# mauro3/KissMCMC.jl

Hardware: AMD Instinct MI355X
Metric: walker-steps/sec (higher is better)
Workload: dtype f64

## Files before the change

### include/kissmcmc_hip.h

```cpp
#ifndef KISSMCMC_HIP_H
#define KISSMCMC_HIP_H

#include <stdint.h>

#ifdef __cplusplus
extern "C" {
#endif

#define KMC_VERSION 100

typedef enum kmc_status {
    KMC_OK = 0,
    KMC_ERR_A_SCALE = 1,
    KMC_ERR_ODD_WALKERS = 2,
    KMC_ERR_TOO_FEW_WALKERS = 3,
    KMC_ERR_BAD_ARG = 4,
    KMC_ERR_NONFINITE_LOGP = 5,
    KMC_ERR_HIP = 6,
    KMC_ERR_OOM = 7,
    KMC_ERR_NO_DEVICE = 8,
    KMC_ERR_UNSUPPORTED = 9
} kmc_status;

typedef enum kmc_density {
// ... 344 lines not shown
                                 int device, double* mean, double* cov, int64_t* n_out, int64_t* info);
kmc_status  kmc_cov_plan(int64_t ncols, int32_t* tile_cols, int32_t* strip_tiles, int32_t* nstrips, int32_t* rows_per_wave_block);
kmc_status  kmc_cov_correlation(int64_t ncols, const double* cov, double* corr, double* sd);

kmc_status  kmc_sampler_pointwise_stats(kmc_sampler* s, int64_t first_sample, const uint8_t* walker_mask ,
                                        int64_t thin, const double* data , int64_t ndata2, int32_t ncols2,
                                        double* stats, int64_t* n_out, int64_t* info);
kmc_status  kmc_chain_pointwise_stats(kmc_user_density* density, const double* params, const double* chain_host ,
                                      int64_t nsamples, int64_t nwalkers, int64_t ndim, int64_t first_sample, const uint8_t* walker_mask,
                                      int64_t thin, const double* data, int64_t ndata2, int32_t ncols2, int device, double* stats,
                                      int64_t* n_out, int64_t* info);
kmc_status  kmc_sampler_pointwise_loglike(kmc_sampler* s, int64_t first_sample, const uint8_t* walker_mask, int64_t thin, const double* data,
                                          int64_t ndata2, int32_t ncols2, int64_t obs_first, int64_t obs_count, double* out, int64_t* n_out);
kmc_status  kmc_chain_pointwise_loglike(kmc_user_density* density, const double* params, const double* chain_host, int64_t nsamples,
                                        int64_t nwalkers, int64_t ndim, int64_t first_sample, const uint8_t* walker_mask, int64_t thin,
                                        const double* data, int64_t ndata2, int32_t ncols2, int64_t obs_first, int64_t obs_count, int device,
                                        double* out, int64_t* n_out);
kmc_status  kmc_pointwise_plan(int64_t n, int64_t ndata, int64_t* run_len, int64_t* nruns, int32_t* lanes_per_run, int32_t* slots,
                               int64_t* nwaves);
kmc_status  kmc_waic_stats(int64_t J, int64_t n, const double* stats, double* lppd_j, double* p_waic_j, double* elpd_j, double* totals);

kmc_status  kmc_sampler_psis_loo(kmc_sampler* s, int64_t first_sample, const uint8_t* walker_mask , int64_t thin,
                                 double r_eff, int64_t obs_first, int64_t obs_count, int64_t workspace_bytes, double* stats, double* lppd_j,
                                 int64_t* n_out, int64_t* info);
kmc_status  kmc_chain_psis_loo(kmc_user_density* density, const double* params, const double* chain_host ,
                               int64_t nsamples, int64_t nwalkers, int64_t ndim, int64_t first_sample, const uint8_t* walker_mask, int64_t thin,
                               double r_eff, int64_t obs_first, int64_t obs_count, int64_t workspace_bytes, int device, double* stats,
                               double* lppd_j, int64_t* n_out, int64_t* info);
kmc_status  kmc_sampler_psis_tail(kmc_sampler* s, int64_t first_sample, const uint8_t* walker_mask, int64_t thin, double r_eff, int64_t obs_first,
                                  int64_t obs_count, int64_t workspace_bytes, double* tail, double* m_j, double* xc_j, int32_t* n_tail_j,
                                  int64_t* tail_len, int64_t* n_out);
kmc_status  kmc_chain_psis_tail(kmc_user_density* density, const double* params, const double* chain_host, int64_t nsamples, int64_t nwalkers,
                                int64_t ndim, int64_t first_sample, const uint8_t* walker_mask, int64_t thin, double r_eff, int64_t obs_first,
                                int64_t obs_count, int64_t workspace_bytes, int device, double* tail, double* m_j, double* xc_j,
                                int32_t* n_tail_j, int64_t* tail_len, int64_t* n_out);
kmc_status  kmc_psis_plan(int64_t n, int64_t ndata, double r_eff, int64_t workspace_bytes, int64_t* tail_len, int64_t* m_est,
                          int64_t* obs_per_block, int64_t* passes);
kmc_status  kmc_loo_stats(int64_t J, int64_t n, const double* stats, const double* lppd_j, double* p_loo_j, double* totals);
kmc_status  kmc_psis_smooth_host(int64_t nt, const double* x, double xc, double* k_hat, double* sigma, double* s, double* sums);

kmc_status  kmc_sampler_relative_eff(kmc_sampler* s, int64_t first_sample, const uint8_t* walker_mask , int64_t thin,
                                     int64_t obs_first, int64_t obs_count, int32_t split, int64_t max_lag, int64_t workspace_bytes,
                                     double* r_eff_j, double* ess_j, int64_t* T_j, int32_t* flags_j, int64_t* m_out, int64_t* h_out, int64_t* n_out,
                                     int64_t* info);
kmc_status  kmc_chain_relative_eff(kmc_user_density* density, const double* params, const double* chain_host ,
                                   int64_t nsamples, int64_t nwalkers, int64_t ndim, int64_t first_sample, const uint8_t* walker_mask, int64_t thin,
                                   int64_t obs_first, int64_t obs_count, int32_t split, int64_t max_lag, int64_t workspace_bytes, int device,
                                   double* r_eff_j, double* ess_j, int64_t* T_j, int32_t* flags_j, int64_t* m_out, int64_t* h_out, int64_t* n_out,
                                   int64_t* info);
kmc_status  kmc_sampler_pointwise_weights(kmc_sampler* s, int64_t first_sample, const uint8_t* walker_mask, int64_t thin, const double* data,
                                          int64_t ndata2, int32_t ncols2, int64_t obs_first, int64_t obs_count, double* v, double* M_j,
                                          int64_t* n_out);
kmc_status  kmc_chain_pointwise_weights(kmc_user_density* density, const double* params, const double* chain_host, int64_t nsamples,
                                        int64_t nwalkers, int64_t ndim, int64_t first_sample, const uint8_t* walker_mask, int64_t thin,
                                        const double* data, int64_t ndata2, int32_t ncols2, int64_t obs_first, int64_t obs_count, int device,
                                        double* v, double* M_j, int64_t* n_out);
kmc_status  kmc_sampler_psis_loo_reff(kmc_sampler* s, int64_t first_sample, const uint8_t* walker_mask, int64_t thin,
                                      const double* r_eff_j , int32_t split, int64_t max_lag, int64_t obs_first,
                                      int64_t obs_count, int64_t workspace_bytes, double* stats, double* lppd_j, double* r_eff_used,
                                      int64_t* tail_len_j, int64_t* n_reff_nan, int64_t* n_out, int64_t* info);
kmc_status  kmc_chain_psis_loo_reff(kmc_user_density* density, const double* params, const double* chain_host, int64_t nsamples, int64_t nwalkers,
                                    int64_t ndim, int64_t first_sample, const uint8_t* walker_mask, int64_t thin, const double* r_eff_j,
                                    int32_t split, int64_t max_lag, int64_t obs_first, int64_t obs_count, int64_t workspace_bytes, int device,
                                    double* stats, double* lppd_j, double* r_eff_used, int64_t* tail_len_j, int64_t* n_reff_nan, int64_t* n_out,
                                    int64_t* info);
kmc_status  kmc_sampler_psis_tail_reff(kmc_sampler* s, int64_t first_sample, const uint8_t* walker_mask, int64_t thin, const double* r_eff_j,
                                       int32_t split, int64_t max_lag, int64_t obs_first, int64_t obs_count, int64_t workspace_bytes, double* tail,
                                       double* m_j, double* xc_j, int32_t* n_tail_j, int64_t* tail_len, double* r_eff_used, int64_t* tail_len_j,
                                       int64_t* n_reff_nan, int64_t* n_out);
kmc_status  kmc_chain_psis_tail_reff(kmc_user_density* density, const double* params, const double* chain_host, int64_t nsamples, int64_t nwalkers,
                                     int64_t ndim, int64_t first_sample, const uint8_t* walker_mask, int64_t thin, const double* r_eff_j,
                                     int32_t split, int64_t max_lag, int64_t obs_first, int64_t obs_count, int64_t workspace_bytes, int device,
                                     double* tail, double* m_j, double* xc_j, int32_t* n_tail_j, int64_t* tail_len, double* r_eff_used,
                                     int64_t* tail_len_j, int64_t* n_reff_nan, int64_t* n_out);

kmc_status  kmc_debug_accept_terms(uint64_t seed, uint64_t step, uint64_t walker0, int64_t n, int64_t nhalf, double a_scale,
                                   int64_t ndim, int device, int64_t* partner_host, double* z_host, double* t1_host, double* lu_host);
kmc_status  kmc_debug_chain_by_walker(const void* src_host, int is_float, int64_t K, int64_t nl, int64_t ld, int64_t nd, int64_t w0,
                                      int64_t nw, int64_t dst_stride, double* dst_host, int64_t dst_len, int device);
kmc_status  kmc_debug_rows_compact(const double* src_host, int64_t rows, int64_t ld, int64_t nd, double* dst_host, int64_t dst_len,
                                   int device);
int         kmc_debug_phase_spec(int density, int L, int K, int iter);
int         kmc_debug_shared_draws(int density, int L, int K, int iter);
int         kmc_debug_replay_variant(int density, int64_t nwalkers, int64_t ndim, int64_t nburnin, int64_t g0, int64_t n, int moments, int chain);

#ifdef __cplusplus
}
#endif
#endif
```

### kissmcmc.jl_amd/_lib.py

```python
from __future__ import annotations

import ctypes as C
import os

_HERE = os.path.dirname(os.path.abspath(__file__))
LIB_PATH = os.environ.get("KMC_LIB_PATH") or os.path.join(_HERE, "libkissmcmc_hip.so")

OK, ERR_A_SCALE, ERR_ODD_WALKERS, ERR_TOO_FEW_WALKERS, ERR_BAD_ARG, ERR_NONFINITE_LOGP, \
    ERR_HIP, ERR_OOM, ERR_NO_DEVICE, ERR_UNSUPPORTED = range(10)
GAUSSIAN_ISO, EXPONENTIAL, ROSENBROCK, LOGNORMAL, MVNORMAL2 = range(5)
USER_DENSITY = 100
HOST_DENSITY = 101
DATA_DENSITY = 102
HOST_LOGPDF_FN = C.CFUNCTYPE(C.c_int, C.POINTER(C.c_double), C.c_int64, C.c_int64, C.POINTER(C.c_double), C.c_void_p)
HOST_PROPOSE_FN = C.CFUNCTYPE(C.c_int, C.POINTER(C.c_double), C.c_int64, C.c_int64, C.POINTER(C.c_double), C.c_void_p)
HOST_ACCEPTED_FN = C.CFUNCTYPE(C.c_int, C.POINTER(C.c_uint8), C.c_int64, C.c_int64, C.c_int64, C.c_int32, C.c_void_p)
F64 = 0
F32 = 1
STORE_CHAIN, STORE_LOGP, MOMENTS, NO_GRAPH, P2P, ISLANDS, P2P_FINEGRAINED, P2P_PUSH = 1, 2, 4, 8, 16, 64, 128, 512
STREAM_CHAIN = 2048
CHAIN_BY_WALKER = 4096
STORE_BLOBS = 8192
MOVE_STRETCH, MOVE_DE, MOVE_SNOOKER, MOVE_MIX = 0, 1, 3, 4
MIX_MAX = 4
TEMPS_MAX = 64
CONV_NEED_LAGS, CONV_TRUNCATED = 1, 2
CONV_HAS_NAN = 4
TEMPER_WHOLE, TEMPER_LIKELIHOOD = 0, 1
P2P_HANDLE_BYTES = 128
RCCL_ID_BYTES = 128

SYMBOLS = [
    "kmc_version", "kmc_device_count", "kmc_last_error", "kmc_status_string", "kmc_validate",
    "kmc_g_pdf", "kmc_cdf_g_inv", "kmc_emcee_run", "kmc_sampler_create", "kmc_sampler_destroy",
    "kmc_sampler_set_stream", "kmc_sampler_bind_positions", "kmc_sampler_p2p_export", "kmc_sampler_p2p_connect", "kmc_sampler_p2p_connect_local", "kmc_sampler_p2p_link_probe", "kmc_sampler_set_positions", "kmc_sampler_init_ball", "kmc_sampler_set_state", "kmc_sampler_run", "kmc_sampler_half_step",
    "kmc_sampler_sync", "kmc_sampler_last_run_ms", "kmc_sampler_generation", "kmc_sampler_nsamples",
    "kmc_sampler_launch_count", "kmc_sampler_describe", "kmc_sampler_device_ptr", "kmc_sampler_get_positions",
    "kmc_sampler_get_logp", "kmc_sampler_get_naccept", "kmc_sampler_get_accept_ratio",
    "kmc_sampler_get_moments", "kmc_sampler_get_chain", "kmc_sampler_get_chain_by_walker", "kmc_logpdf_eval", "kmc_logpdf_eval_host",
    "kmc_user_density_create", "kmc_user_density_create_body", "kmc_user_density_destroy", "kmc_metropolis_validate", "kmc_metropolis_run", "kmc_cholesky_lower", "kmc_int_acorr", "kmc_sampler_int_acorr",
    "kmc_sizeof_config", "kmc_sizeof_metropolis_config", "kmc_sizeof_outputs", "kmc_sizeof_metropolis_outputs", "kmc_deal_seed", "kmc_deal_perm", "kmc_sampler_deal_pack", "kmc_sampler_deal_unpack",
    "kmc_sampler_get_walker_ids", "kmc_sampler_set_walker_ids", "kmc_sampler_set_chain_host", "kmc_rccl_unique_id", "kmc_sampler_rccl_init",
    "kmc_sampler_rccl_capture", "kmc_sampler_rccl_set_capture", "kmc_rccl_version", "kmc_device_free_bytes",
    "kmc_sampler_launch_mode", "kmc_updated_budget", "kmc_set_updated_budget_mb", "kmc_debug_accept_terms",
    "kmc_debug_chain_by_walker", "kmc_debug_rows_compact", "kmc_debug_phase_spec", "kmc_debug_shared_draws", "kmc_debug_replay_variant",
    "kmc_user_density_create_body_blob", "kmc_user_density_nblob", "kmc_logpdf_blob_eval_host", "kmc_sampler_get_blobs",
    "kmc_device_cache_release", "kmc_user_density_is_separable", "kmc_host_prefault", "kmc_data_density_create",
    "kmc_sampler_get_rung_state", "kmc_sampler_set_rung_state", "kmc_sampler_get_swaps",
    "kmc_sampler_get_rung_loglike", "kmc_sampler_set_rung_loglike_sum", "kmc_sampler_get_ladder", "kmc_sampler_set_ladder",
    "kmc_sampler_order_stats", "kmc_sampler_chain_argmax", "kmc_chain_order_stats", "kmc_chain_argmax",
    "kmc_sampler_histograms", "kmc_chain_histograms", "kmc_hist_pair_plan",
    "kmc_sampler_lag_sums", "kmc_chain_lag_sums", "kmc_convergence_stats", "kmc_sampler_convergence", "kmc_chain_convergence",
    "kmc_convergence_plan",
    "kmc_rank_plan", "kmc_rank_normal_scores", "kmc_sampler_rank_scores", "kmc_chain_rank_scores", "kmc_sampler_rank_convergence",
    "kmc_chain_rank_convergence",
    "kmc_sampler_hdi", "kmc_chain_hdi", "kmc_hdi_span",
    "kmc_sampler_covariance", "kmc_chain_covariance", "kmc_cov_plan", "kmc_cov_correlation",
    "kmc_sampler_pointwise_stats", "kmc_chain_pointwise_stats", "kmc_sampler_pointwise_loglike", "kmc_chain_pointwise_loglike",
    "kmc_pointwise_plan", "kmc_waic_stats",
    "kmc_sampler_psis_loo", "kmc_chain_psis_loo", "kmc_sampler_psis_tail", "kmc_chain_psis_tail", "kmc_psis_plan", "kmc_loo_stats",
    "kmc_psis_smooth_host",
    "kmc_sampler_relative_eff", "kmc_chain_relative_eff", "kmc_sampler_pointwise_weights", "kmc_chain_pointwise_weights",
    "kmc_sampler_psis_loo_reff", "kmc_chain_psis_loo_reff", "kmc_sampler_psis_tail_reff", "kmc_chain_psis_tail_reff",
]


class Config(C.Structure):
    _fields_ = [
        ("dtype", C.c_int32),
        ("density", C.c_int32),
        ("params", C.c_double * 8),
        ("nwalkers", C.c_int64),
        ("ndim", C.c_int64),
        ("ngenerations", C.c_int64),
        ("nburnin", C.c_int64),
        ("nthin", C.c_int64),
        ("a_scale", C.c_double),
        ("seed", C.c_uint64),
        ("flags", C.c_uint32),
        ("device", C.c_int32),
        ("shard_rank", C.c_int32),
        ("shard_count", C.c_int32),
        ("user_density", C.c_void_p),
        ("island_gens", C.c_int32),
        ("island_size", C.c_int32),
        ("host_logpdf", C.c_void_p),
        ("host_user", C.c_void_p),
        ("host_accepted", C.c_void_p),
        ("deal_rank", C.c_int32),
        ("deal_count", C.c_int32),
        ("temper_mode", C.c_int32),
        ("temper_pad_", C.c_int32),
        ("adapt_until", C.c_int64),
        ("adapt_lag", C.c_double),
        ("adapt_time", C.c_double),
        ("adapt", C.c_int32),
        ("adapt_pad_", C.c_int32),
        ("snooker_gamma", C.c_double),
        ("mix_count", C.c_int32),
        ("mix_move0", C.c_int32), ("mix_move1", C.c_int32), ("mix_move2", C.c_int32), ("mix_move3", C.c_int32),
        ("mix_pad0_", C.c_int32), ("mix_pad1_", C.c_int32), ("mix_pad2_", C.c_int32),
        ("mix_weight0", C.c_double), ("mix_weight1", C.c_double), ("mix_weight2", C.c_double), ("mix_weight3", C.c_double),
        ("mix_gamma0", C.c_double), ("mix_gamma1", C.c_double), ("mix_gamma2", C.c_double), ("mix_gamma3", C.c_double),
        ("mix_sigma0", C.c_double), ("mix_sigma1", C.c_double), ("mix_sigma2", C.c_double), ("mix_sigma3", C.c_double),
        ("betas", C.c_void_p),
        ("ntemps", C.c_int32),
        ("swap_every", C.c_int32),
        ("move", C.c_int32),
        ("move_pad_", C.c_int32),
        ("de_gamma0", C.c_double),
        ("de_sigma", C.c_double),
    ]


class Outputs(C.Structure):
    _fields_ = [
        ("chain", C.POINTER(C.c_double)),
        ("chain_logp", C.POINTER(C.c_double)),
        ("accept_ratio", C.POINTER(C.c_double)),
        ("naccept", C.POINTER(C.c_int64)),
        ("final_pos", C.POINTER(C.c_double)),
        ("final_logp", C.POINTER(C.c_double)),
        ("sum", C.POINTER(C.c_double)),
        ("sumsq", C.POINTER(C.c_double)),
        ("nmoment", C.c_int64),
        ("nsamples", C.c_int64),
        ("device_ms", C.c_double),
        ("blobs", C.POINTER(C.c_double)),
# ... 147 lines not shown
    L.kmc_sampler_chain_argmax.argtypes = [vp, C.c_int64, bp, ip, ip, dp, dp]
    L.kmc_chain_order_stats.argtypes = [dp, dp, C.c_int64, C.c_int64, C.c_int64, C.c_int64, bp, ip, C.c_int32, C.c_int, dp, dp, ip]
    L.kmc_chain_argmax.argtypes = [dp, dp, C.c_int64, C.c_int64, C.c_int64, C.c_int64, bp, C.c_int, ip, ip, dp, dp]
    i32p = C.POINTER(C.c_int32)
    L.kmc_sampler_histograms.argtypes = [vp, C.c_int64, bp, i32p, C.c_int32, dp, C.c_int32, C.c_int32, ip, ip, ip, ip]
    L.kmc_chain_histograms.argtypes = [dp, dp, C.c_int64, C.c_int64, C.c_int64, C.c_int64, bp, i32p, C.c_int32, dp, C.c_int32, C.c_int, ip, ip, ip, ip]
    L.kmc_hist_pair_plan.argtypes = [C.c_int32, C.c_int32, i32p, i32p, i32p]
    L.kmc_sampler_lag_sums.argtypes = [vp, C.c_int64, bp, C.c_int32, C.c_int32, C.c_int64, C.c_int64, dp, dp, dp, ip, ip]
    L.kmc_chain_lag_sums.argtypes = [dp, dp, C.c_int64, C.c_int64, C.c_int64, C.c_int64, bp, C.c_int32, C.c_int64, C.c_int64, C.c_int, dp, dp, dp, ip, ip]
    L.kmc_convergence_stats.argtypes = [C.c_int64, C.c_int64, C.c_int64, dp, dp, dp, C.c_int64, C.c_int64, dp, dp, dp, dp, dp, dp, dp, ip, i32p]
    L.kmc_sampler_convergence.argtypes = [vp, C.c_int64, bp, C.c_int32, C.c_int32, C.c_int64, dp, dp, dp, dp, dp, dp, dp, ip, i32p, ip, ip, ip]
    L.kmc_chain_convergence.argtypes = [dp, dp, C.c_int64, C.c_int64, C.c_int64, C.c_int64, bp, C.c_int32, C.c_int64, C.c_int, dp, dp, dp, dp, dp, dp, dp, ip, i32p, ip, ip, ip]
    L.kmc_convergence_plan.argtypes = [i32p, i32p, i32p, i32p]
    L.kmc_rank_plan.argtypes = [i32p, i32p, i32p, i32p]
    L.kmc_rank_normal_scores.argtypes = [ip, C.c_int64, C.c_int64, dp]
    L.kmc_sampler_rank_scores.argtypes = [vp, C.c_int64, bp, C.c_int32, C.c_int32, C.c_int32, ip, dp, dp, ip, ip, ip]
    L.kmc_chain_rank_scores.argtypes = [dp, dp, C.c_int64, C.c_int64, C.c_int64, C.c_int64, bp, C.c_int32, C.c_int32, C.c_int, ip, dp, dp, ip, ip, ip]
    L.kmc_sampler_rank_convergence.argtypes = [vp, C.c_int64, bp, C.c_int32, C.c_int32, C.c_int64] + [dp] * 10 + [ip, i32p, ip, ip, ip]
    L.kmc_chain_rank_convergence.argtypes = [dp, dp, C.c_int64, C.c_int64, C.c_int64, C.c_int64, bp, C.c_int32, C.c_int64, C.c_int] + [dp] * 10 + [ip, i32p, ip, ip, ip]
    L.kmc_sampler_hdi.argtypes = [vp, C.c_int64, bp, C.c_int32, dp, C.c_int32, dp, dp, ip, ip, ip, ip]
    L.kmc_chain_hdi.argtypes = [dp, dp, C.c_int64, C.c_int64, C.c_int64, C.c_int64, bp, dp, C.c_int32, C.c_int, dp, dp, ip, ip, ip, ip]
    L.kmc_hdi_span.argtypes = [C.c_int64, C.c_double, ip, ip]
    L.kmc_sampler_covariance.argtypes = [vp, C.c_int64, bp, C.c_int32, dp, dp, ip, ip]
    L.kmc_chain_covariance.argtypes = [dp, dp, C.c_int64, C.c_int64, C.c_int64, C.c_int64, bp, C.c_int, dp, dp, ip, ip]
    L.kmc_cov_plan.argtypes = [C.c_int64, i32p, i32p, i32p, i32p]
    L.kmc_cov_correlation.argtypes = [C.c_int64, dp, dp, dp]
    held_out = [dp, C.c_int64, C.c_int32]
    host_chain = [vp, dp, dp, C.c_int64, C.c_int64, C.c_int64, C.c_int64, bp, C.c_int64]
    L.kmc_sampler_pointwise_stats.argtypes = [vp, C.c_int64, bp, C.c_int64] + held_out + [dp, ip, ip]
    L.kmc_chain_pointwise_stats.argtypes = host_chain + held_out + [C.c_int, dp, ip, ip]
    L.kmc_sampler_pointwise_loglike.argtypes = [vp, C.c_int64, bp, C.c_int64] + held_out + [C.c_int64, C.c_int64, dp, ip]
    L.kmc_chain_pointwise_loglike.argtypes = host_chain + held_out + [C.c_int64, C.c_int64, C.c_int, dp, ip]
    L.kmc_pointwise_plan.argtypes = [C.c_int64, C.c_int64, ip, ip, i32p, i32p, ip]
    L.kmc_waic_stats.argtypes = [C.c_int64, C.c_int64, dp, dp, dp, dp, dp]
    psis_sel = [C.c_double, C.c_int64, C.c_int64, C.c_int64]
    L.kmc_sampler_psis_loo.argtypes = [vp, C.c_int64, bp, C.c_int64] + psis_sel + [dp, dp, ip, ip]
    L.kmc_chain_psis_loo.argtypes = host_chain + psis_sel + [C.c_int, dp, dp, ip, ip]
    L.kmc_sampler_psis_tail.argtypes = [vp, C.c_int64, bp, C.c_int64] + psis_sel + [dp, dp, dp, i32p, ip, ip]
    L.kmc_chain_psis_tail.argtypes = host_chain + psis_sel + [C.c_int, dp, dp, dp, i32p, ip, ip]
    L.kmc_psis_plan.argtypes = [C.c_int64, C.c_int64, C.c_double, C.c_int64, ip, ip, ip, ip]
    L.kmc_loo_stats.argtypes = [C.c_int64, C.c_int64, dp, dp, dp, dp]
    L.kmc_psis_smooth_host.argtypes = [C.c_int64, dp, C.c_double, dp, dp, dp, dp]
    reff_sel = [C.c_int64, C.c_int64, C.c_int32, C.c_int64, C.c_int64]
    L.kmc_sampler_relative_eff.argtypes = [vp, C.c_int64, bp, C.c_int64] + reff_sel + [dp, dp, ip, i32p, ip, ip, ip, ip]
    L.kmc_chain_relative_eff.argtypes = host_chain + reff_sel + [C.c_int, dp, dp, ip, i32p, ip, ip, ip, ip]
    L.kmc_sampler_pointwise_weights.argtypes = [vp, C.c_int64, bp, C.c_int64] + held_out + [C.c_int64, C.c_int64, dp, dp, ip]
    L.kmc_chain_pointwise_weights.argtypes = host_chain + held_out + [C.c_int64, C.c_int64, C.c_int, dp, dp, ip]
    psis_reff = [dp, C.c_int32, C.c_int64, C.c_int64, C.c_int64, C.c_int64]
    L.kmc_sampler_psis_loo_reff.argtypes = [vp, C.c_int64, bp, C.c_int64] + psis_reff + [dp, dp, dp, ip, ip, ip, ip]
    L.kmc_chain_psis_loo_reff.argtypes = host_chain + psis_reff + [C.c_int, dp, dp, dp, ip, ip, ip, ip]
    L.kmc_sampler_psis_tail_reff.argtypes = [vp, C.c_int64, bp, C.c_int64] + psis_reff + [dp, dp, dp, i32p, ip, dp, ip, ip, ip]
    L.kmc_chain_psis_tail_reff.argtypes = host_chain + psis_reff + [C.c_int, dp, dp, dp, i32p, ip, dp, ip, ip, ip]
    L.kmc_deal_seed.restype = C.c_uint64
    L.kmc_deal_seed.argtypes = [C.c_uint64, C.c_int32]
    L.kmc_deal_perm.argtypes = [C.c_uint64, C.c_int64, C.c_int32, C.c_int64, ip, ip]
    L.kmc_sampler_deal_pack.argtypes = [vp, C.c_int64, vp]
    L.kmc_sampler_deal_unpack.argtypes = [vp, vp]
    L.kmc_sampler_get_walker_ids.argtypes = [vp, ip]
    L.kmc_sampler_set_walker_ids.argtypes = [vp, ip]
    L.kmc_sampler_set_chain_host.argtypes = [vp, dp, dp]
    L.kmc_rccl_unique_id.argtypes = [vp]
    L.kmc_sampler_rccl_init.argtypes = [vp, vp]
    L.kmc_sampler_rccl_capture.argtypes = [vp, C.POINTER(C.c_int)]
    L.kmc_sampler_rccl_set_capture.argtypes = [vp, C.c_int]
    L.kmc_rccl_version.argtypes = [C.POINTER(C.c_int), C.c_char_p, C.c_int64]
    L.kmc_device_free_bytes.argtypes = [C.c_int, C.POINTER(C.c_uint64), C.POINTER(C.c_uint64)]
    L.kmc_device_cache_release.argtypes = []
    L.kmc_device_cache_release.restype = None
    L.kmc_host_prefault.argtypes = [C.c_void_p, C.c_uint64, C.c_int]
    L.kmc_host_prefault.restype = None
    L.kmc_sampler_launch_mode.restype = C.c_int
    L.kmc_sampler_launch_mode.argtypes = [vp, C.POINTER(C.c_int)]
    L.kmc_updated_budget.restype = None
    L.kmc_updated_budget.argtypes = [ip, ip]
    L.kmc_set_updated_budget_mb.restype = None
    L.kmc_set_updated_budget_mb.argtypes = [C.c_double]
    L.kmc_debug_accept_terms.argtypes = [C.c_uint64, C.c_uint64, C.c_uint64, C.c_int64, C.c_int64, C.c_double, C.c_int64, C.c_int, ip, dp, dp, dp]
    L.kmc_debug_chain_by_walker.argtypes = [vp, C.c_int, C.c_int64, C.c_int64, C.c_int64, C.c_int64, C.c_int64, C.c_int64, C.c_int64, dp, C.c_int64, C.c_int]
    L.kmc_debug_rows_compact.argtypes = [dp, C.c_int64, C.c_int64, C.c_int64, dp, C.c_int64, C.c_int]
    L.kmc_debug_phase_spec.restype = C.c_int
    L.kmc_debug_phase_spec.argtypes = [C.c_int, C.c_int, C.c_int, C.c_int]
    L.kmc_debug_shared_draws.restype = C.c_int
    L.kmc_debug_shared_draws.argtypes = [C.c_int, C.c_int, C.c_int, C.c_int]
    L.kmc_debug_replay_variant.restype = C.c_int
    L.kmc_debug_replay_variant.argtypes = [C.c_int, C.c_int64, C.c_int64, C.c_int64, C.c_int64, C.c_int64, C.c_int, C.c_int]
    for fn, T in ((L.kmc_sizeof_config, Config), (L.kmc_sizeof_metropolis_config, MetropolisConfig),
                  (L.kmc_sizeof_outputs, Outputs), (L.kmc_sizeof_metropolis_outputs, MetropolisOutputs)):
        if fn() != C.sizeof(T):
            raise ImportError(f"{LIB_PATH}: struct layout mismatch ({fn.__name__}() = {fn()}, the ctypes mirror {T.__name__} is {C.sizeof(T)} bytes): "
                              "rebuild the library or update kissmcmc_jl_amd/_lib.py from include/kissmcmc_hip.h")
    _lib = L
    return L


def check(status: int) -> None:
    if status != OK:
        L = lib()
        msg = L.kmc_last_error().decode() or L.kmc_status_string(status).decode()
        raise KmcError(status, msg)
```

### kissmcmc.jl_amd/csrc/kmc_plan.hip

```cpp
#include <algorithm>
#include <cmath>
#include <cstdlib>
#include <cstring>

#include "kmc_sampler.hpp"

using namespace kmc;
using namespace kmc_host;

namespace kmc_host {
bool lookup(int density, int L, int K, int iter, bool p2p, bool ragged, bool f32, HalfStepFn* vec, HalfStepFn* gen)
{
    return with_density(density, false, [&](auto d) {
        using D = decltype(d);
        if (p2p && f32) { *vec = nullptr; *gen = nullptr; }
        else if (p2p) density_part<D, 2>(L, K, iter, ragged, false, vec, gen);
        else if (ragged || f32) density_part<D, 1>(L, K, iter, ragged, f32, vec, gen);
        else density_part<D, 0>(L, K, iter, false, false, vec, gen);
        return true;
    });
}

bool lookup_move(int move, int density, int L, int K, int iter, bool ragged, HalfStepFn* vec, HalfStepFn* gen)
{
    return with_density(density, false, [&](auto d) {
        if (move == KMC_MOVE_SNOOKER) density_part<decltype(d), 4>(L, K, iter, ragged, false, vec, gen);
        else if (move == KMC_MOVE_MIX) density_part<decltype(d), 5>(L, K, iter, ragged, false, vec, gen);
        else density_part<decltype(d), 3>(L, K, iter, ragged, false, vec, gen);
        return true;
    });
}

bool lookup_temper(int move, int density, int L, int K, int iter, bool ragged, HalfStepFn* vec, HalfStepFn* gen)
{
    return with_density(density, false, [&](auto d) {
        using D = decltype(d);
        if (move == KMC_MOVE_SNOOKER) temper_part<D, Move::Snooker>(L, K, iter, ragged, vec, gen);
        else if (move == KMC_MOVE_MIX) temper_part<D, Move::Mix>(L, K, iter, ragged, vec, gen);
        else if (move == KMC_MOVE_DE) temper_part<D, Move::DE>(L, K, iter, ragged, vec, gen);
        else temper_part<D, Move::Stretch>(L, K, iter, ragged, vec, gen);
        return true;
    });
}

HalfStepFn lookup_spec(int density, int L, int K, int iter)
{
    return with_density(density, HalfStepFn(nullptr), [&](auto d) { return spec_part<decltype(d)>(L, K, iter); });
}

HalfStepFn lookup_share(int density, int L, int K, int iter, int* share)
{
    *share = 0;
    return with_density(density, HalfStepFn(nullptr), [&](auto d) -> HalfStepFn {
        if constexpr (std::is_same<decltype(d), MvNormal2>::value) return nullptr;
        else return share_part<decltype(d)>(L, K, iter, share);
    });
}

LogpdfFn logpdf_fn(int density)
{
    return with_density(density, LogpdfFn(nullptr), [](auto d) { return logpdf_lookup<decltype(d)>(); });
}

bool resident_lane_wanted(int64_t ndim)
{
    std::string e;
    if (debug_opt("resident", &e) && e == "pair") return false;
    return ndim <= 8;
}
int lane_nd(int64_t ndim) { return (int)ndim; }

void philox_host(const uint32_t ctr[4], const uint32_t key[2], uint32_t out[4])
{
    uint32_t c0 = ctr[0], c1 = ctr[1], c2 = ctr[2], c3 = ctr[3], k0 = key[0], k1 = key[1];
    for (int r = 0; r < 10; ++r) {
        const uint64_t p0 = (uint64_t)0xD2511F53u * c0, p1 = (uint64_t)0xCD9E8D57u * c2;
        const uint32_t n0 = (uint32_t)(p1 >> 32) ^ c1 ^ k0, n2 = (uint32_t)(p0 >> 32) ^ c3 ^ k1;
        c0 = n0; c1 = (uint32_t)p1; c2 = n2; c3 = (uint32_t)p0;
        k0 += 0x9E3779B9u; k1 += 0xBB67AE85u;
    }
    out[0] = c0; out[1] = c1; out[2] = c2; out[3] = c3;
}

static void affine_perm(const uint32_t ctr[4], uint64_t seed, int64_t n, int64_t* A, int64_t* C)
{
    const uint32_t key[2] = {(uint32_t)seed, (uint32_t)(seed >> 32)};
    uint32_t w[4];
    philox_host(ctr, key, w);
    auto gcd = [](int64_t a, int64_t b) { while (b) { const int64_t t = a % b; a = b; b = t; } return a; };
    int64_t a = (int64_t)((((uint64_t)w[0] << 32) | w[1]) % (uint64_t)n);
    if (a < 1) a = 1;
    while (gcd(a, n) != 1) a = (a + 1 >= n) ? 1 : a + 1;
    *A = a;
    *C = (int64_t)((((uint64_t)w[2] << 32) | w[3]) % (uint64_t)n);
}

void island_perm(uint64_t seed, int64_t epoch, int64_t N, int64_t* A, int64_t* C)
{
    if (epoch == 0 || N <= 2) { *A = 1; *C = 0; return; }
    const uint32_t ctr[4] = {(uint32_t)epoch, (uint32_t)((uint64_t)epoch >> 32), 0x49534c41u, 0u};
    affine_perm(ctr, seed, N, A, C);
}

constexpr uint64_t kDealSeedStride = 0x9E3779B97F4A7C15ull;
uint64_t deal_seed(uint64_t seed, int32_t rank) { return seed + (uint64_t)(rank + 1) * kDealSeedStride; }
void deal_perm(uint64_t seed, int64_t epoch, int32_t rank, int64_t S, int64_t* A, int64_t* C)
{
    const uint32_t ctr[4] = {(uint32_t)epoch, (uint32_t)((uint64_t)epoch >> 32), 0x4445414cu, (uint32_t)rank};
    affine_perm(ctr, seed, S, A, C);
}

Plan make_plan(const kmc_config& c, int64_t n_active)
{
    Plan p;
    HalfStepFn vec = nullptr, gen = nullptr;
    int L = 0, K = 0, iter = 1;
    const char* env = std::getenv("KMC_PLAN");
    bool force_generic = false;
    if (env && std::strcmp(env, "generic") == 0) force_generic = true;
    else if (env && std::sscanf(env, "%d,%d,%d", &L, &K, &iter) == 3) {  }
    else {
        L = 0;
        const int64_t chunks = (c.ndim + 1) / 2;
        auto pow2ceil = [](int64_t v) { int p = 1; while (p < v) p <<= 1; return p; };
        if (chunks <= 4) { L = pow2ceil(chunks); K = 1; }
        else if (chunks <= 128) { L = pow2ceil((chunks + 1) / 2); K = 2; }
        else if (chunks <= 256) { L = 64; K = 4; }
        else if (chunks <= 512) { L = 64; K = 8; }
        if (c.density == KMC_USER_DENSITY && chunks > 64 && chunks <= 128) {
            const kmc_user_density* ud = static_cast<const kmc_user_density*>(c.user_density);
            if (ud && ud->is_body && !sep_routed(ud) && body_vec_possible(ud, c.ndim)) { L = 16; K = 8; }
        }
        iter = 1;
        if (L > 0) {
            const int64_t waves1 = n_active * L / 64;
            if (2 <= L && 2 * K <= 16 && waves1 >= 3072) iter = 2;
            while (iter >= 2 && iter * 2 <= L && iter * 2 * K <= 16 && waves1 / (iter * 2) >= 4096 && iter < 16) iter *= 2;
        }
    }
    const bool de = own_stream_move(c);
    const int tile_cap = c.move == KMC_MOVE_DE ? 8 : 4;
    if (de && (!env || c.move != KMC_MOVE_DE)) while (iter > 1 && iter * K > tile_cap) iter /= 2;
    const bool ragged = L > 0 && 2 * L * K != c.ndim;
    const bool f32 = c.dtype == KMC_F32;
    if ((ragged || f32) && iter > 4) iter = 4;
    if (tempered(c) && iter > 8) iter = 8;
    if ((c.flags & KMC_P2P) && iter > 8) iter = 8;
    p.ragged = ragged;
    if (c.density == KMC_HOST_DENSITY || c.density == KMC_DATA_DENSITY) {
        p.fn = c.move == KMC_MOVE_MIX ? half_step_host_mix() : c.move == KMC_MOVE_SNOOKER ? half_step_host_snooker() : de ? half_step_host_de() : half_step_host(); p.vec = false; p.ragged = false; p.L = 1; p.K = 1; p.ITER = 1;
        if (tempered(c)) {
            if (c.move == KMC_MOVE_SNOOKER) temper_part<HostEval, Move::Snooker>(1, 1, 1, false, &vec, &p.fn);
            else if (c.move == KMC_MOVE_MIX) temper_part<HostEval, Move::Mix>(1, 1, 1, false, &vec, &p.fn);
            else if (c.move == KMC_MOVE_DE) temper_part<HostEval, Move::DE>(1, 1, 1, false, &vec, &p.fn);
            else temper_part<HostEval, Move::Stretch>(1, 1, 1, false, &vec, &p.fn);
        }
        return p;
    }
    if (c.density == KMC_USER_DENSITY) {
        const kmc_user_density* ud = static_cast<const kmc_user_density*>(c.user_density);
        const bool body = ud && ud->is_body && !(sep_routed(ud) || body_vec_possible(ud, c.ndim));
        if (!body && !force_generic && L > 0 && 2 * L * K >= c.ndim && iter <= L && iter * K <= 16) {
            if (ud && ud->is_body && !sep_routed(ud)) while (iter > 1 && body_vec_lds_bytes(L, K, iter) > 65536) iter /= 2;
            p.vec = true; p.L = L; p.K = K; p.ITER = iter;
        } else {
            p.vec = false; p.L = 1; p.K = 1; p.ITER = 1;
        }
        return p;
    }
    if (tempered(c)) lookup_temper(c.move, c.density, L, K, iter, ragged, &vec, &gen);
    else if (de) lookup_move(c.move, c.density, L, K, iter, ragged, &vec, &gen);
    else lookup(c.density, L, K, iter, (c.flags & KMC_P2P) != 0, ragged, f32, &vec, &gen);
    if (!force_generic && L > 0 && 2 * L * K >= c.ndim && vec != nullptr) {
        p.fn = vec; p.vec = true; p.L = L; p.K = K; p.ITER = iter;
        if (!tempered(c) && !de && !(c.flags & KMC_P2P) && !ragged && !f32 && iter <= 2) {
            p.fn_credit = lookup_spec(c.density, L, K, iter);
            p.fn_share_burnin = lookup_share(c.density, L, K, iter, &p.share_burnin);
        }
    } else {
        p.fn = gen; p.vec = false; p.L = 1; p.K = 1; p.ITER = 1;
    }
    return p;
}

kmc_status check_ndim(int density, int64_t ndim)
{
    if (density == KMC_ROSENBROCK && ndim < 2) return fail(KMC_ERR_BAD_ARG, "rosenbrock needs ndim >= 2");
    if (density == KMC_MVNORMAL2 && ndim != 2) return fail(KMC_ERR_BAD_ARG, "mvnormal2 needs ndim == 2");
    return KMC_OK;
}

}
kmc_status kmc_host::digest_params(const kmc_config& c, DensityParams* dp)
{
    for (double& v : dp->p) v = 0.0;
    dp->ndim = (int32_t)c.ndim;
    dp->pad_ = 0;
    const double* p = c.params;
    switch (c.density) {
    case KMC_USER_DENSITY:
        if (!c.user_density) return fail(KMC_ERR_BAD_ARG, "KMC_USER_DENSITY needs kmc_config.user_density");
        for (int i = 0; i < 6; ++i) dp->p[i] = p[i];
        return KMC_OK;
    case KMC_HOST_DENSITY:
        return KMC_OK;
    case KMC_DATA_DENSITY:
        if (!c.user_density) return fail(KMC_ERR_BAD_ARG, "KMC_DATA_DENSITY needs kmc_config.user_density");
        for (int i = 0; i < 6; ++i) dp->p[i] = p[i];
        return KMC_OK;
    case KMC_GAUSSIAN_ISO:
        if (!(p[1] > 0.0)) return fail(KMC_ERR_BAD_ARG, "gaussian: sigma must be > 0");
        dp->p[0] = p[0]; dp->p[1] = 1.0 / p[1];
        return KMC_OK;
    case KMC_EXPONENTIAL:
        if (!(p[0] > 0.0)) return fail(KMC_ERR_BAD_ARG, "exponential: rate must be > 0");
        dp->p[0] = p[0];
        return KMC_OK;
    case KMC_ROSENBROCK:
        if (!(p[2] > 0.0)) return fail(KMC_ERR_BAD_ARG, "rosenbrock: scale must be > 0");
        dp->p[0] = p[0]; dp->p[1] = p[1]; dp->p[2] = 1.0 / p[2];
        return KMC_OK;
    case KMC_LOGNORMAL:
        if (!(p[1] > 0.0)) return fail(KMC_ERR_BAD_ARG, "lognormal: sigma must be > 0");
        dp->p[0] = p[0]; dp->p[1] = p[1];
        return KMC_OK;
    case KMC_MVNORMAL2:
        for (int i = 0; i < 5; ++i) dp->p[i] = p[i];
        return KMC_OK;
    default:
        return fail(KMC_ERR_BAD_ARG, "unknown density id");
    }
}

KMC_EXPORT int kmc_debug_phase_spec(int density, int L, int K, int iter)
{
    return kmc_host::lookup_spec(density, L, K, iter) != nullptr ? 1 : 0;
}

KMC_EXPORT int kmc_debug_shared_draws(int density, int L, int K, int iter)
{
    int share = 0;
    return kmc_host::lookup_share(density, L, K, iter, &share) != nullptr ? share : 0;
}
```

### kissmcmc.jl_amd/csrc/kmc_shared_draws.hpp

```cpp
#pragma once
#include "kmc_tables.hpp"

namespace kmc {

constexpr int kShareRound = 256;

template <class Dens, int L, int K, int ITER, int SHARE>
__device__ __forceinline__ void half_step_share_body(const HalfStepFront& f, const HalfStepArgs& a)
{
    static_assert(BlobTrait<Dens>::n == 0 && RowEvalTrait<Dens>::n == 0, "menu densities with a fragment form");
    static_assert(ITER <= 2, "one or two walkers per group");
    static_assert(SHARE == 2 && SHARE * ITER <= L, "two waves per workgroup (the leader rule below is written for two); the leader's lanes must cover every sibling's walkers");
    constexpr int G = 64 / L;
    constexpr int W = G * ITER;
    constexpr int TPB = 64 * SHARE;
    constexpr int64_t ld = 2 * L * K;
    __shared__ uint32_t sh_partner[SHARE][W];
    __shared__ double sh_z[SHARE][W], sh_t1[SHARE][W], sh_lu[SHARE][W];
    double* const posT = f.pos;
    const int tid   = blockIdx.x * TPB + threadIdx.x;
    const int lane  = threadIdx.x & 63;
    const int wv    = __builtin_amdgcn_readfirstlane((int)(threadIdx.x >> 6));
    const int j     = lane & (L - 1);
    const int g     = lane / L;
// ... 49 lines not shown
    DrawConsts dc = a.dc;
    dc.seed_lo = f.seed_lo; dc.seed_hi = f.seed_hi; dc.nhalf = f.nhalf;
    KMC_STAMP(3);
    double zL = 0.0, t1L = 0.0, luL = 0.0, ua = 0.5;
    if (wv == lead) {
        const double uz = ((double)bits.y + 0.5) * 0x1.0p-32;
        const double t  = fma(uz, dc.c1, dc.c0);
        zL = t * t;
        const uint64_t kk = ((uint64_t)bits.z << 20) | (uint64_t)(bits.w >> 12);
        ua = ((double)kk + 0.5) * 0x1.0p-52;
        t1L = dc.nm1 * log_pos_normal(zL);
    }
    __builtin_amdgcn_sched_barrier(0);
#pragma unroll
    for (int it = kFirst; it < ITER; ++it) load_partner_rows(it);
    __builtin_amdgcn_sched_barrier(0);
    if (wv == lead) {
        luL = log_pos_normal(ua);
        if (pubL) { sh_z[vL][sL] = zL; sh_t1[vL][sL] = t1L; sh_lu[vL][sL] = luL; }
    }
    lds_barrier();
    KMC_STAMP(4);
    Draw dr;
    dr.partner = 0u; dr.z = 0.0; dr.t1 = sh_t1[wv][js * G + g]; dr.lu = sh_lu[wv][js * G + g];
    double zB[ITER];
#pragma unroll
    for (int it = 0; it < ITER; ++it) zB[it] = sh_z[wv][it * G + g];

    double myp1 = 0.0;
#pragma unroll
    for (int it = 0; it < ITER; ++it) {
#pragma unroll
        for (int k = 0; k < K; ++k) {
            xo[it][k].x = fma(zB[it], xc[it][k].x - xo[it][k].x, xo[it][k].x);
            xo[it][k].y = fma(zB[it], xc[it][k].y - xo[it][k].y, xo[it][k].y);
        }
        if constexpr (MultiSumTrait<Dens>::n > 0) {
            double S[MultiSumTrait<Dens>::n];
            Dens::template frag_partial_n<L, K>(xo[it], j, 2 * L * K, a.dp, S);
#pragma unroll
            for (int q = 0; q < MultiSumTrait<Dens>::n; ++q) S[q] = group_sum<L>(S[q]);
            const double p1 = Dens::finish_n(S, a.dp);
            myp1 = (j == it) ? p1 : myp1;
        } else {
            const double S  = group_sum<L>(Dens::template frag_partial<L, K>(xo[it], j, 2 * L * K, a.dp));
            const double p1 = Dens::finish(S, a.dp);
            myp1 = (j == it) ? p1 : myp1;
        }
    }
    KMC_STAMP(5);

    const bool acc = useA && accept_test(dr, myp1, p0);
    const unsigned long long accmask = __ballot(acc);
    if (acc) store_wt(&f.logp[rowA], myp1);
    KMC_STAMP(6);

#pragma unroll
    for (int it = 0; it < ITER; ++it) {
        const bool accB = ((accmask >> (gbase + it)) & 1ull) != 0;
        if (accB) {
            double2* own = reinterpret_cast<double2*>(posT + (own_row0 + w0 + it * G + g) * ld);
#pragma unroll
            for (int k = 0; k < K; ++k) store_row(&own[k * L + j], xo[it][k]);
        }
    }
    KMC_STAMP(7);
#ifdef KMC_PROBE
    {
        unsigned long long st[8];
        asm volatile("s_waitcnt lgkmcnt(0)" ::: "memory");
        KMC_STAMP_READ(st[0], 80, 81); KMC_STAMP_READ(st[1], 82, 83); KMC_STAMP_READ(st[2], 84, 85); KMC_STAMP_READ(st[3], 86, 87);
        KMC_STAMP_READ(st[4], 88, 89); KMC_STAMP_READ(st[5], 90, 91); KMC_STAMP_READ(st[6], 92, 93); KMC_STAMP_READ(st[7], 94, 95);
        if (lane == 0 && (tid >> 6) < 8192) for (int q = 0; q < 8; q += (KMC_PROBE == 2 ? 7 : 1)) g_probe[half][tid >> 6][q] = st[q];
    }
#endif
}

template <class Dens, int L, int K, int ITER, int SHARE>
__global__ __launch_bounds__(64 * SHARE) void half_step_vec_share(KMC_FRONT_PARAMS, const HalfStepArgs a)
{
    half_step_share_body<Dens, L, K, ITER, SHARE>(KMC_FRONT_PACK, a);
}

constexpr int kShareWaves = 2;

#ifdef KMC_TABLES_IMPL
template <class D>
HalfStepFn share_part(int L, int K, int iter, int* share)
{
    *share = 0;
    if constexpr (D::kHasFrag && BlobTrait<D>::n == 0 && RowEvalTrait<D>::n == 0) {
        if (L == 8 && K == 2 && iter == 2) {
            *share = kShareWaves;
            return half_step_vec_share<D, 8, 2, 2, kShareWaves>;
        }
    }
    return nullptr;
}
#define KMC_INSTANTIATE_SHARE(D) template HalfStepFn share_part<D>(int, int, int, int*)
#endif

}
```

### kissmcmc.jl_amd/csrc/kmc_tables.hpp

```cpp
#pragma once
#include <type_traits>
#include "kmc_islands.hpp"
#include "kmc_generation.hpp"
#include "kmc_metropolis.hpp"

namespace kmc {

using HalfStepFn = void (*)(KMC_FRONT_TYPES, const HalfStepArgs);
using LogpdfFn = void (*)(const LogpdfArgs);
using FlushFn = void (*)(const FlushArgs);
using IslandFn = void (*)(const IslandArgs);
using ResidentFn = void (*)(const ResidentArgs);
using GenerationFn = void (*)(KMC_GEN_FRONT_TYPES, const GenerationArgs);
using InitBallFn = void (*)(const InitBallArgs);
using MetropolisFn = void (*)(const MetropolisArgs);
using MetropolisTabledFn = void (*)(const MetropolisArgs, const double*, int);

template <class D, int PART> void density_part(int L, int K, int iter, bool ragged, bool f32, HalfStepFn* vec, HalfStepFn* gen);
template <class D, Move M> void temper_part(int L, int K, int iter, bool ragged, HalfStepFn* vec, HalfStepFn* gen);
template <class D> HalfStepFn spec_part(int L, int K, int iter);
template <class D> HalfStepFn share_part(int L, int K, int iter, int* share);
template <class D> LogpdfFn logpdf_lookup();
template <class D> InitBallFn init_ball_lookup();
template <class D> IslandFn island_lookup(int S, int K, bool ragged);
template <class D> ResidentFn resident_lookup(int tpb, int K, bool ragged);
template <class D> ResidentFn resident_lane_lookup(int ndim, bool f32);
template <class D> ResidentFn resident_lane2_lookup(int ndim);
template <class D> GenerationFn generation_lane_lookup(int ndim);
template <class D> GenerationFn generation_group_lookup(int L, int K);
template <class D> MetropolisFn metropolis_lookup(int ndim);
template <class D> MetropolisTabledFn metropolis_tabled_lookup(int ndim);
template <class D> MetropolisFn metropolis_mv_lookup(int ndim);
HalfStepFn half_step_host();
HalfStepFn half_step_host_de();
HalfStepFn half_step_host_snooker();
HalfStepFn half_step_host_mix();

#ifdef KMC_TABLES_IMPL
template <class D, int L, int K, int ITER, bool P2P, bool RAGGED, class T, Move M>
HalfStepFn vec_one()
{
    if constexpr (ITER > L || ITER * K > 16 || ((M == Move::Snooker || M == Move::Mix) && ITER > 1 && ITER * K > 4)) return nullptr;
    else if constexpr (M == Move::Snooker) return half_step_snooker_vec<D, L, K, ITER, RAGGED>;
    else if constexpr (M == Move::Mix) return half_step_mix_vec<D, L, K, ITER, RAGGED>;
    else if constexpr (M == Move::DE) return half_step_de_vec<D, L, K, ITER, RAGGED>;
    else return half_step_vec<D, L, K, ITER, P2P, RAGGED, T>;
}

template <class D, int L, int K, bool P2P, bool RAGGED, class T, Move M = Move::Stretch>
HalfStepFn vec_iter(int iter)
{
    constexpr bool kWide = !P2P && !RAGGED && sizeof(T) == 8;
    switch (iter) {
    case 1: return vec_one<D, L, K, 1, P2P, RAGGED, T, M>();
    case 2: return vec_one<D, L, K, 2, P2P, RAGGED, T, M>();
    case 4: return vec_one<D, L, K, 4, P2P, RAGGED, T, M>();
    case 8: if constexpr (kWide || (P2P && !RAGGED)) return vec_one<D, L, K, 8, P2P, RAGGED, T, M>(); else return nullptr;
    case 16: if constexpr (kWide) return vec_one<D, L, K, 16, P2P, RAGGED, T, M>(); else return nullptr;
    default: return nullptr;
    }
}

template <class D, int L, int K, int PART>
HalfStepFn vec_pick(int iter, bool ragged, bool f32)
{
    if constexpr (PART == 0) return vec_iter<D, L, K, false, false, double>(iter);
    else if constexpr (PART == 1) {
        if (f32) return ragged ? vec_iter<D, L, K, false, true, float>(iter) : vec_iter<D, L, K, false, false, float>(iter);
        return vec_iter<D, L, K, false, true, double>(iter);
    } else if constexpr (PART == 2) return ragged ? vec_iter<D, L, K, true, true, double>(iter) : vec_iter<D, L, K, true, false, double>(iter);
    else if constexpr (PART == 3) return ragged ? vec_iter<D, L, K, false, true, double, Move::DE>(iter) : vec_iter<D, L, K, false, false, double, Move::DE>(iter);
    else if constexpr (PART == 4) return ragged ? vec_iter<D, L, K, false, true, double, Move::Snooker>(iter) : vec_iter<D, L, K, false, false, double, Move::Snooker>(iter);
    else return ragged ? vec_iter<D, L, K, false, true, double, Move::Mix>(iter) : vec_iter<D, L, K, false, false, double, Move::Mix>(iter);
}

template <class D, int PART>
HalfStepFn vec_lookup(int L, int K, int iter, bool ragged, bool f32)
{
    if constexpr (!D::kHasFrag) {
        return nullptr;
    } else {
#define KMC_LK(l, k) if (L == l && K == k) return vec_pick<D, l, k, PART>(iter, ragged, f32);
        KMC_LK(1, 1) KMC_LK(2, 1) KMC_LK(4, 1) KMC_LK(4, 2) KMC_LK(8, 2) KMC_LK(16, 2) KMC_LK(32, 2) KMC_LK(64, 2)
        KMC_LK(64, 4) KMC_LK(64, 8)
#undef KMC_LK
        if constexpr (PART == 0 && std::is_same<D, GaussianIso>::value) {
#define KMC_LK(l, k) if (L == l && K == k) return vec_iter<D, l, k, false, false, double>(iter);
            KMC_LK(8, 1) KMC_LK(16, 1) KMC_LK(32, 1) KMC_LK(64, 1) KMC_LK(4, 4) KMC_LK(8, 4)
#undef KMC_LK
        }
        return nullptr;
    }
}

template <class D, int PART>
void density_part(int L, int K, int iter, bool ragged, bool f32, HalfStepFn* vec, HalfStepFn* gen)
{
    *vec = vec_lookup<D, PART>(L, K, iter, ragged, f32);
    if constexpr (PART == 0) *gen = half_step_generic<D, false, double>;
    else if constexpr (PART == 1) *gen = f32 ? half_step_generic<D, false, float> : half_step_generic<D, false, double>;
    else if constexpr (PART == 2) *gen = half_step_generic<D, true, double>;
    else if constexpr (PART == 3) *gen = half_step_de_generic<D>;
    else if constexpr (PART == 4) *gen = half_step_snooker_generic<D>;
    else *gen = half_step_mix_generic<D>;
// ... 221 lines not shown
```

Measured before the change: 9.079 billion.

## Add four-lane-per-walker shared-draw burn-in kernel for separable menu densities

Adds a shared-draw half-step variant where each walker row (ndim 32) is handled by 4 lanes holding 4 double2 each, instead of 8 lanes with two iterations. One wave per workgroup alternately computes RNG draws and publishes them via LDS to both waves. It is selected by default for GaussianIso, Exponential and LogNormal in the burn-in share path, with a debug option to disable it. The change aims to cut the per-walker RNG and log work and the iteration overhead, at the cost of more registers per lane and a different reduction layout.

```diff
diff --git a/include/kissmcmc_hip.h b/include/kissmcmc_hip.h
--- a/include/kissmcmc_hip.h
+++ b/include/kissmcmc_hip.h
@@ -450,6 +450,7 @@
                                    int device);
 int         kmc_debug_phase_spec(int density, int L, int K, int iter);
 int         kmc_debug_shared_draws(int density, int L, int K, int iter);
+int         kmc_debug_shared_draws_lanes(int density, int L, int K, int iter);
 int         kmc_debug_replay_variant(int density, int64_t nwalkers, int64_t ndim, int64_t nburnin, int64_t g0, int64_t n, int moments, int chain);
 
 #ifdef __cplusplus
diff --git a/kissmcmc.jl_amd/_lib.py b/kissmcmc.jl_amd/_lib.py
--- a/kissmcmc.jl_amd/_lib.py
+++ b/kissmcmc.jl_amd/_lib.py
@@ -43,7 +43,7 @@
     "kmc_sampler_get_walker_ids", "kmc_sampler_set_walker_ids", "kmc_sampler_set_chain_host", "kmc_rccl_unique_id", "kmc_sampler_rccl_init",
     "kmc_sampler_rccl_capture", "kmc_sampler_rccl_set_capture", "kmc_rccl_version", "kmc_device_free_bytes",
     "kmc_sampler_launch_mode", "kmc_updated_budget", "kmc_set_updated_budget_mb", "kmc_debug_accept_terms",
-    "kmc_debug_chain_by_walker", "kmc_debug_rows_compact", "kmc_debug_phase_spec", "kmc_debug_shared_draws", "kmc_debug_replay_variant",
+    "kmc_debug_chain_by_walker", "kmc_debug_rows_compact", "kmc_debug_phase_spec", "kmc_debug_shared_draws", "kmc_debug_shared_draws_lanes", "kmc_debug_replay_variant",
     "kmc_user_density_create_body_blob", "kmc_user_density_nblob", "kmc_logpdf_blob_eval_host", "kmc_sampler_get_blobs",
     "kmc_device_cache_release", "kmc_user_density_is_separable", "kmc_host_prefault", "kmc_data_density_create",
     "kmc_sampler_get_rung_state", "kmc_sampler_set_rung_state", "kmc_sampler_get_swaps",
@@ -357,6 +357,8 @@
     L.kmc_debug_phase_spec.argtypes = [C.c_int, C.c_int, C.c_int, C.c_int]
     L.kmc_debug_shared_draws.restype = C.c_int
     L.kmc_debug_shared_draws.argtypes = [C.c_int, C.c_int, C.c_int, C.c_int]
+    L.kmc_debug_shared_draws_lanes.restype = C.c_int
+    L.kmc_debug_shared_draws_lanes.argtypes = [C.c_int, C.c_int, C.c_int, C.c_int]
     L.kmc_debug_replay_variant.restype = C.c_int
     L.kmc_debug_replay_variant.argtypes = [C.c_int, C.c_int64, C.c_int64, C.c_int64, C.c_int64, C.c_int64, C.c_int, C.c_int]
     for fn, T in ((L.kmc_sizeof_config, Config), (L.kmc_sizeof_metropolis_config, MetropolisConfig),
diff --git a/kissmcmc.jl_amd/csrc/kmc_plan.hip b/kissmcmc.jl_amd/csrc/kmc_plan.hip
--- a/kissmcmc.jl_amd/csrc/kmc_plan.hip
+++ b/kissmcmc.jl_amd/csrc/kmc_plan.hip
@@ -48,12 +48,15 @@
     return with_density(density, HalfStepFn(nullptr), [&](auto d) { return spec_part<decltype(d)>(L, K, iter); });
 }
 
-HalfStepFn lookup_share(int density, int L, int K, int iter, int* share)
+HalfStepFn lookup_share(int density, int L, int K, int iter, int* share, int* lanes)
 {
     *share = 0;
+    *lanes = 0;
+    std::string v;
+    const int rows4 = (debug_opt("rows4", &v) && v == "0") ? 0 : 1;
     return with_density(density, HalfStepFn(nullptr), [&](auto d) -> HalfStepFn {
         if constexpr (std::is_same<decltype(d), MvNormal2>::value) return nullptr;
-        else return share_part<decltype(d)>(L, K, iter, share);
+        else return share_part<decltype(d)>(L, K, iter, rows4, share, lanes);
     });
 }
 
@@ -175,7 +178,8 @@
         p.fn = vec; p.vec = true; p.L = L; p.K = K; p.ITER = iter;
         if (!tempered(c) && !de && !(c.flags & KMC_P2P) && !ragged && !f32 && iter <= 2) {
             p.fn_credit = lookup_spec(c.density, L, K, iter);
-            p.fn_share_burnin = lookup_share(c.density, L, K, iter, &p.share_burnin);
+            int lanes = 0;
+            p.fn_share_burnin = lookup_share(c.density, L, K, iter, &p.share_burnin, &lanes);
         }
     } else {
         p.fn = gen; p.vec = false; p.L = 1; p.K = 1; p.ITER = 1;
@@ -239,6 +243,12 @@
 
 KMC_EXPORT int kmc_debug_shared_draws(int density, int L, int K, int iter)
 {
-    int share = 0;
-    return kmc_host::lookup_share(density, L, K, iter, &share) != nullptr ? share : 0;
-}
+    int share = 0, lanes = 0;
+    return kmc_host::lookup_share(density, L, K, iter, &share, &lanes) != nullptr ? share : 0;
+}
+
+KMC_EXPORT int kmc_debug_shared_draws_lanes(int density, int L, int K, int iter)
+{
+    int share = 0, lanes = 0;
+    return kmc_host::lookup_share(density, L, K, iter, &share, &lanes) != nullptr ? lanes : 0;
+}
diff --git a/kissmcmc.jl_amd/csrc/kmc_shared_draws.hpp b/kissmcmc.jl_amd/csrc/kmc_shared_draws.hpp
--- a/kissmcmc.jl_amd/csrc/kmc_shared_draws.hpp
+++ b/kissmcmc.jl_amd/csrc/kmc_shared_draws.hpp
@@ -155,22 +155,142 @@
     half_step_share_body<Dens, L, K, ITER, SHARE>(KMC_FRONT_PACK, a);
 }
 
+template <class D> struct Rows4Trait { static constexpr bool ok = false; };
+template <> struct Rows4Trait<GaussianIso> { static constexpr bool ok = true; };
+template <> struct Rows4Trait<Exponential> { static constexpr bool ok = true; };
+template <> struct Rows4Trait<LogNormal>   { static constexpr bool ok = true; };
+
+template <class Dens, int SHARE>
+__device__ __forceinline__ void half_step_rows4_body(const HalfStepFront& f, const HalfStepArgs& a)
+{
+    static_assert(Rows4Trait<Dens>::ok && BlobTrait<Dens>::n == 0 && RowEvalTrait<Dens>::n == 0 && MultiSumTrait<Dens>::n == 0, "menu densities whose fragment is a sum of per-element terms");
+    static_assert(SHARE == 2, "two waves per workgroup (the leader rule below is written for two)");
+    constexpr int L = 4, K = 4, W = 16;
+    constexpr int TPB = 64 * SHARE;
+    constexpr int64_t ld = 2 * L * K;
+    __shared__ uint32_t sh_partner[SHARE][W];
+    __shared__ double sh_z[SHARE][W], sh_t1[SHARE][W], sh_lu[SHARE][W];
+    double* const posT = f.pos;
+    const int tid   = blockIdx.x * TPB + threadIdx.x;
+    const int lane  = threadIdx.x & 63;
+    const int wv    = __builtin_amdgcn_readfirstlane((int)(threadIdx.x >> 6));
+    const int j     = lane & (L - 1);
+    const int g     = lane / L;
+    const int w0    = (tid >> 6) * W;
+    const int half  = f.half();
+    const int64_t own_row0 = (int64_t)f.gw0;
+    const int64_t oth_row0 = (int64_t)(1 - half) * (int64_t)f.nhalf;
+    const int lead = (int)(((unsigned)blockIdx.x / (2u * (unsigned)kShareRound)) & 1u);
+    KMC_STAMP(0);
+
+    const int64_t rowA = own_row0 + w0 + g;
+    double2 xc[K], xo[K];
+    {
+        const double2* own = reinterpret_cast<const double2*>(posT + rowA * ld);
+#pragma unroll
+        for (int k = 0; k < K; ++k) xc[k] = load_row(&own[k * L + j]);
+    }
+    const double p0 = f.logp[rowA];
+    __builtin_amdgcn_sched_barrier(0);
+
+    const bool pubL = j < SHARE;
+    const uint64_t step = (uint64_t)f.step;
+    DrawConsts dcf{};
+    dcf.seed_lo = f.seed_lo; dcf.seed_hi = f.seed_hi; dcf.nhalf = f.nhalf;
+    U4 bits{0u, 0u, 0u, 0u};
+    if (wv == lead) {
+        const int iL = ((int)blockIdx.x * SHARE + (pubL ? j : SHARE - 1)) * W + g;
+        bits = draw_bits(dcf, step, (uint64_t)f.gw0 + (uint64_t)iL);
+        if (pubL) sh_partner[j][g] = draw_partner(dcf, bits);
+    }
+    lds_barrier();
+    KMC_STAMP(1);
+    {
+        const uint32_t partner = sh_partner[wv][g];
+        const double2* oth = reinterpret_cast<const double2*>(posT + (oth_row0 + partner) * ld);
+#pragma unroll
+        for (int k = 0; k < K; ++k) xo[k] = load_row(&oth[k * L + j]);
+    }
+    __builtin_amdgcn_sched_barrier(0);
+    KMC_STAMP(2);
+
+    DrawConsts dc = a.dc;
+    dc.seed_lo = f.seed_lo; dc.seed_hi = f.seed_hi; dc.nhalf = f.nhalf;
+    KMC_STAMP(3);
+    if (wv == lead) {
+        const double uz = ((double)bits.y + 0.5) * 0x1.0p-32;
+        const double t  = fma(uz, dc.c1, dc.c0);
+        const double zL = t * t;
+        const uint64_t kk = ((uint64_t)bits.z << 20) | (uint64_t)(bits.w >> 12);
+        const double ua = ((double)kk + 0.5) * 0x1.0p-52;
+        const double t1L = dc.nm1 * log_pos_normal(zL);
+        const double luL = log_pos_normal(ua);
+        if (pubL) { sh_z[j][g] = zL; sh_t1[j][g] = t1L; sh_lu[j][g] = luL; }
+    }
+    lds_barrier();
+    KMC_STAMP(4);
+    Draw dr;
+    dr.partner = 0u; dr.z = 0.0; dr.t1 = sh_t1[wv][g]; dr.lu = sh_lu[wv][g];
+    const double z = sh_z[wv][g];
+
+#pragma unroll
+    for (int k = 0; k < K; ++k) {
+        xo[k].x = fma(z, xc[k].x - xo[k].x, xo[k].x);
+        xo[k].y = fma(z, xc[k].y - xo[k].y, xo[k].y);
+    }
+    const double2 ylo[2] = {xo[0], xo[2]}, yhi[2] = {xo[1], xo[3]};
+    const double Slo = group_sum<4>(Dens::template frag_partial<8, 2>(ylo, j, 2 * L * K, a.dp));
+    const double Shi = group_sum<4>(Dens::template frag_partial<8, 2>(yhi, j + 4, 2 * L * K, a.dp));
+    const double p1  = Dens::finish(Slo + Shi, a.dp);
+    KMC_STAMP(5);
+
+    const bool acc = accept_test(dr, p1, p0);
+    if (acc && j == 0) store_wt(&f.logp[rowA], p1);
+    KMC_STAMP(6);
+    if (acc) {
+        double2* own = reinterpret_cast<double2*>(posT + rowA * ld);
+#pragma unroll
+        for (int k = 0; k < K; ++k) store_row(&own[k * L + j], xo[k]);
+    }
+    KMC_STAMP(7);
+#ifdef KMC_PROBE
+    {
+        unsigned long long st[8];
+        asm volatile("s_waitcnt lgkmcnt(0)" ::: "memory");
+        KMC_STAMP_READ(st[0], 80, 81); KMC_STAMP_READ(st[1], 82, 83); KMC_STAMP_READ(st[2], 84, 85); KMC_STAMP_READ(st[3], 86, 87);
+        KMC_STAMP_READ(st[4], 88, 89); KMC_STAMP_READ(st[5], 90, 91); KMC_STAMP_READ(st[6], 92, 93); KMC_STAMP_READ(st[7], 94, 95);
+        if (lane == 0 && (tid >> 6) < 8192) for (int q = 0; q < 8; q += (KMC_PROBE == 2 ? 7 : 1)) g_probe[half][tid >> 6][q] = st[q];
+    }
+#endif
+}
+
+template <class Dens, int SHARE>
+__global__ __launch_bounds__(64 * SHARE) void half_step_vec_share_rows4(KMC_FRONT_PARAMS, const HalfStepArgs a)
+{
+    half_step_rows4_body<Dens, SHARE>(KMC_FRONT_PACK, a);
+}
+
 constexpr int kShareWaves = 2;
 
 #ifdef KMC_TABLES_IMPL
 template <class D>
-HalfStepFn share_part(int L, int K, int iter, int* share)
+HalfStepFn share_part(int L, int K, int iter, int rows4, int* share, int* lanes)
 {
     *share = 0;
+    *lanes = 0;
     if constexpr (D::kHasFrag && BlobTrait<D>::n == 0 && RowEvalTrait<D>::n == 0) {
         if (L == 8 && K == 2 && iter == 2) {
             *share = kShareWaves;
+            if constexpr (Rows4Trait<D>::ok) {
+                if (rows4 != 0) { *lanes = 4; return half_step_vec_share_rows4<D, kShareWaves>; }
+            }
+            *lanes = 8;
             return half_step_vec_share<D, 8, 2, 2, kShareWaves>;
         }
     }
     return nullptr;
 }
-#define KMC_INSTANTIATE_SHARE(D) template HalfStepFn share_part<D>(int, int, int, int*)
+#define KMC_INSTANTIATE_SHARE(D) template HalfStepFn share_part<D>(int, int, int, int, int*, int*)
 #endif
 
 }
diff --git a/kissmcmc.jl_amd/csrc/kmc_tables.hpp b/kissmcmc.jl_amd/csrc/kmc_tables.hpp
--- a/kissmcmc.jl_amd/csrc/kmc_tables.hpp
+++ b/kissmcmc.jl_amd/csrc/kmc_tables.hpp
@@ -19,7 +19,7 @@
 template <class D, int PART> void density_part(int L, int K, int iter, bool ragged, bool f32, HalfStepFn* vec, HalfStepFn* gen);
 template <class D, Move M> void temper_part(int L, int K, int iter, bool ragged, HalfStepFn* vec, HalfStepFn* gen);
 template <class D> HalfStepFn spec_part(int L, int K, int iter);
-template <class D> HalfStepFn share_part(int L, int K, int iter, int* share);
+template <class D> HalfStepFn share_part(int L, int K, int iter, int rows4, int* share, int* lanes);
 template <class D> LogpdfFn logpdf_lookup();
 template <class D> InitBallFn init_ball_lookup();
 template <class D> IslandFn island_lookup(int S, int K, bool ragged);
```

Result: no change. 9.148 billion (median of 6 runs) (+0.8%).
